# felipemcoelho/nf4-triton-dequantization

Hardware: AMD Instinct MI355X
Metric: dequantized elements/s (4096x4096 NF4->bf16, blocksize 64 / nested 256) (higher is better)
Workload: dtype f32

## Files before the change

nf4_triton_dequantization_amd/csrc/nf4_dequant.hip:

```cpp
#include <hip/hip_runtime.h>
#include <stdint.h>

#include "../../include/nf4_dequant.h"
#include "nf4_common.h"

namespace {

using namespace nf4dq;

enum Mode : int { kRef = 0, kSingle = 1, kBnb = 2, kBnbSingle = 3 };

struct Desc {
    const uint32_t* packed;
    const uint8_t* a1;
    const float* a2;
    const float* code2;
    u32x4* out;
    float offset;
    uint32_t nbytes;
    uint32_t tile_begin;
    uint32_t groups;
    FastDiv nb;
    FastDiv n2;
    FastDiv bpr;
    uint32_t blk_shift;
    uint32_t blk2_shift;
    uint32_t blk_base;
};

#ifndef NF4_FLAT_STAMPS
#define NF4_FLAT_STAMPS 0
#endif

template <int MAXB>
struct Batch {
    Desc d[MAXB];
    uint32_t count;
    uint32_t total_tiles;
#if NF4_FLAT_STAMPS
    unsigned long long* stamps;
#endif
};

#if NF4_FLAT_STAMPS
#define NF4_FSTAMP(slot_, val_)                                                                      \
    do {                                                                                             \
        __builtin_amdgcn_sched_barrier(0);                                                           \
        if (lane == 0) bt.stamps[(blockIdx.x * kFlatWaves + (threadIdx.x >> 6)) * 4u + (slot_)] = (val_); \
        __builtin_amdgcn_sched_barrier(0);                                                           \
    } while (0)
#define NF4_FNOW() __builtin_amdgcn_s_memrealtime()
#else
#define NF4_FSTAMP(slot_, val_) \
    do {                        \
    } while (0)
#define NF4_FNOW() 0ull
#endif

template <int DT>
__device__ __forceinline__ void store1(void* out, int64_t i, float x) {
    if constexpr (DT == NF4DQ_BF16) {
        reinterpret_cast<__bf16*>(out)[i] = (__bf16)x;
    } else if constexpr (DT == NF4DQ_F16) {
        reinterpret_cast<_Float16*>(out)[i] = (_Float16)opaque(x);
    } else {
        reinterpret_cast<float*>(out)[i] = x;
    }
}

#ifndef NF4_DQ_FLAT_WAVES
#define NF4_DQ_FLAT_WAVES 4
#endif
#ifndef NF4_DQ_U
#define NF4_DQ_U 4
#endif
#ifndef NF4_DQ_AUX_STORE
#define NF4_DQ_AUX_STORE 18
#endif
#ifndef NF4_DQ_AUX_LOAD
#define NF4_DQ_AUX_LOAD 2
#endif
#ifndef NF4_DQ_SCALE_FIRST
#define NF4_DQ_SCALE_FIRST 0
#endif
#ifndef NF4_DQ_SCALE_NT
#define NF4_DQ_SCALE_NT 0
#endif
#ifndef NF4_DQ_DECODE
#define NF4_DQ_DECODE 1
#endif
#ifndef NF4_DQ_SINGLE_FAST
#define NF4_DQ_SINGLE_FAST 1
#endif
#ifndef NF4_DQ_ABL_NOSCALE
#define NF4_DQ_ABL_NOSCALE 0
#endif



constexpr int kWg = 256;
constexpr int kFlatWaves = NF4_DQ_FLAT_WAVES;
constexpr int kFlatWg = 64 * kFlatWaves;
constexpr int kU = NF4_DQ_U;

constexpr int kAuxStore = NF4_DQ_AUX_STORE;
constexpr int kAuxLoad = NF4_DQ_AUX_LOAD;

template <int DT>
constexpr uint32_t out_bytes_per_packed_byte() { return DT == NF4DQ_F32 ? 8u : 4u; }
template <int DT>
constexpr uint32_t lane_bytes() { return DT == NF4DQ_F32 ? 2u : 4u; }
template <int DT>
constexpr uint32_t tile_bytes() { return 64u * lane_bytes<DT>() * kU; }

struct TileIn {
    uint32_t w[kU];
    uint32_t a1;
    float a2;
};

template <int DT>
__device__ __forceinline__ uint32_t tile_block(const Desc& D, uint32_t base, uint32_t lane) {
    constexpr uint32_t kTileBytes = tile_bytes<DT>();
    const uint32_t bsh = D.blk_shift;
    const uint32_t bpt = kTileBytes >> bsh;
    uint32_t g = (base >> bsh) + (bpt ? (lane & (bpt - 1u)) : 0u);
    const uint32_t nblk = (D.nbytes + (1u << bsh) - 1u) >> bsh;
    g = g < nblk ? g : nblk - 1u;
    return g + D.blk_base;
}

template <int DT, int MODE>
__device__ __forceinline__ TileIn tile_load(const Desc& D, __amdgpu_buffer_rsrc_t rp, uint32_t base, uint32_t lane) {
    constexpr uint32_t LB = lane_bytes<DT>();
    TileIn in;
    auto packed_loads = [&]() {
#pragma unroll
        for (int j = 0; j < kU; ++j) {
            const uint32_t off = base + 64u * LB * j + LB * lane;
            if constexpr (LB == 4) {
                in.w[j] = __builtin_amdgcn_raw_buffer_load_b32(rp, off, 0, kAuxLoad);
            } else {
                in.w[j] = __builtin_amdgcn_raw_buffer_load_b16(rp, off, 0, kAuxLoad);
            }
        }
    };
    if constexpr (!NF4_DQ_SCALE_FIRST) packed_loads();
    const uint32_t g = tile_block<DT>(D, base, lane);
    if constexpr (NF4_DQ_ABL_NOSCALE) {
        in.a1 = g & 255u;
        in.a2 = 0.01f;
    } else if constexpr (MODE == kRef) {
        const uint32_t r = fdiv(g, D.bpr);
        const uint32_t b = g - r * D.bpr.d;
        const uint8_t* pa1 = D.a1 + fmodu(g, D.nb);
        const float* pa2 = D.a2 + fmodu(r * D.groups + (b >> 2), D.n2);
        if constexpr (NF4_DQ_SCALE_NT) {
            in.a1 = __builtin_nontemporal_load(pa1);
            in.a2 = __builtin_nontemporal_load(pa2);
        } else {
            in.a1 = *pa1;
            in.a2 = *pa2;
        }
    } else if constexpr (MODE == kSingle) {
        const uint32_t r = fdiv(g, D.bpr);
        const uint32_t b = g - r * D.bpr.d;
        in.a2 = D.a2[r * D.n2.d + b];
    } else if constexpr (MODE == kBnb) {
        in.a1 = D.a1[g];
        in.a2 = D.a2[g >> D.blk2_shift];
    } else {
        in.a2 = D.a2[g];
    }
    if constexpr (NF4_DQ_SCALE_FIRST) packed_loads();
    return in;
}

template <int DT, int MODE>
__device__ __forceinline__ void tile_finish(const Desc& D, __amdgpu_buffer_rsrc_t ro, const float* lut,
                                            const TileIn& in, uint32_t base, uint32_t lane, const float* code2s) {
    float s;
    if constexpr (MODE == kRef) {
        s = ((float)in.a1 / 127.0f) * in.a2;
    } else if constexpr (MODE == kBnb) {
        s = code2s[in.a1] * in.a2 + D.offset;
    } else {
        s = in.a2;
    }
    const uint32_t bsh = D.blk_shift;
    constexpr uint32_t kOB = out_bytes_per_packed_byte<DT>();
    constexpr uint32_t LB = lane_bytes<DT>();
#pragma unroll
    for (int j = 0; j < kU; ++j) {
        const uint32_t rel = 64u * LB * j + LB * lane;
        const float sj = __shfl(s, (int)(rel >> bsh), 64);
        const uint32_t w = in.w[j];
        const uint32_t hi4 = (w >> 2) & 0x3C3C3C3Cu;
        const uint32_t lo4 = (w << 2) & 0x3C3C3C3Cu;
        const char* t = reinterpret_cast<const char*>(lut);
        float v[2 * LB];
#pragma unroll
        for (int k = 0; k < (int)LB; ++k) {
            v[2 * k] = *reinterpret_cast<const float*>(t + ((hi4 >> (8 * k)) & 0xFFu)) * sj;
            v[2 * k + 1] = *reinterpret_cast<const float*>(t + ((lo4 >> (8 * k)) & 0xFFu)) * sj;
        }
        const uint32_t ob = (base + rel) * kOB;
        if constexpr (DT == NF4DQ_F32) {
            u32x4 o = {__float_as_uint(v[0]), __float_as_uint(v[1]), __float_as_uint(v[2]), __float_as_uint(v[3])};
            __builtin_amdgcn_raw_buffer_store_b128(o, ro, ob, 0, kAuxStore);
        } else {
            u32x4 o = {pack2<DT>(v[0], v[1]), pack2<DT>(v[2], v[3]), pack2<DT>(v[4], v[5]), pack2<DT>(v[6], v[7])};
            __builtin_amdgcn_raw_buffer_store_b128(o, ro, ob, 0, kAuxStore);
        }
    }
}

typedef uint16_t __attribute__((may_alias)) u16_alias;
typedef uint32_t __attribute__((may_alias)) u32_alias;
typedef uint32_t u32x4_alias __attribute__((ext_vector_type(4), may_alias));

struct TblCtx {
    char* tbl;
    uint32_t tb;
    f32x2 c01;
};

template <int DT, int MODE>
__device__ __forceinline__ void tile_finish_tbl(const Desc& D, __amdgpu_buffer_rsrc_t ro, const TileIn& in,
                                                uint32_t base, uint32_t lane, const float* code2s,
                                                const TblCtx& c) {
    float s;
    if constexpr (MODE == kRef) {
        s = ((float)in.a1 / 127.0f) * in.a2;
    } else if constexpr (MODE == kBnb) {
        s = code2s[in.a1] * in.a2 + D.offset;
    } else {
        s = in.a2;
    }
    const uint32_t bsh = D.blk_shift;
    const uint32_t k = lane & 7u;
#pragma unroll
    for (int j = 0; j < kU; ++j) {
        const uint32_t rel = 256u * j + 4u * lane;
        const float sj = __shfl(s, (int)(rel >> bsh), 64);
        *reinterpret_cast<u32_alias*>(c.tbl + c.tb + 4u * k) = pack2<DT>(c.c01.x * sj, c.c01.y * sj);
        const uint32_t w = in.w[j];
        const uint32_t hb = (w >> 3) & 0x1E1E1E1Eu;
        const uint32_t lb = (w << 1) & 0x1E1E1E1Eu;
        uint32_t o[4];
#pragma unroll
        for (int b = 0; b < 4; ++b) {
            const uint32_t ah = __builtin_amdgcn_perm(hb, c.tb, 0x03020104u + b);
            const uint32_t al = __builtin_amdgcn_perm(lb, c.tb, 0x03020104u + b);
            const uint32_t vh = *reinterpret_cast<const u16_alias*>(c.tbl + ah);
            const uint32_t vl = *reinterpret_cast<const u16_alias*>(c.tbl + al);
            o[b] = vh | (vl << 16);
        }
        const u32x4 ov = {o[0], o[1], o[2], o[3]};
        __builtin_amdgcn_raw_buffer_store_b128(ov, ro, (base + rel) * 4u, 0, kAuxStore);
    }
}

template <int MAXB>
__device__ __forceinline__ uint32_t find_matrix(const Batch<MAXB>& bt, uint32_t t, uint32_t k) {
    if constexpr (MAXB > 1) {
        while (k + 1 < bt.count && t >= bt.d[k + 1].tile_begin) ++k;
    }
    return k;
}

struct Cursor {
    uint32_t t, k, base;
    bool valid;
};

template <int DT, int MAXB>
__device__ __forceinline__ Cursor cursor_at(const Batch<MAXB>& bt, uint32_t t, uint32_t k_hint) {
    constexpr uint32_t kTileBytes = tile_bytes<DT>();
    Cursor c;
    c.t = t;
    c.valid = t < bt.total_tiles;
    c.k = c.valid ? find_matrix(bt, t, k_hint) : k_hint;
    c.base = c.valid ? (t - bt.d[c.k].tile_begin) * kTileBytes : 0xFFFFF000u;
    return c;
}

template <int DT, int MAXB>
__device__ __forceinline__ void make_rsrcs(const Batch<MAXB>& bt, uint32_t k, __amdgpu_buffer_rsrc_t& rp,
                                           __amdgpu_buffer_rsrc_t& ro) {
    constexpr uint32_t kOB = out_bytes_per_packed_byte<DT>();
    rp = __builtin_amdgcn_make_buffer_rsrc((void*)bt.d[k].packed, 0, bt.d[k].nbytes, kRsrcFlags);
    ro = __builtin_amdgcn_make_buffer_rsrc((void*)bt.d[k].out, 0, bt.d[k].nbytes * kOB, kRsrcFlags);
}

template <int DT, int MODE, int MAXB>
__global__ __launch_bounds__(kFlatWg) void nf4_flat_kernel(const Batch<MAXB> bt) {
    __shared__ __attribute__((aligned(16))) float lut[16];
    __shared__ __attribute__((aligned(16))) float code2s[MODE == kBnb ? 256 : 1];
    constexpr bool kTbl = NF4_DQ_DECODE == 1 && DT != NF4DQ_F32;
    __shared__ __attribute__((aligned(256))) char tbl[kTbl ? kFlatWaves * 2048 : 4];
    const uint32_t lane = threadIdx.x & 63u;
#if NF4_FLAT_STAMPS
    const unsigned long long t_entry = NF4_FNOW();
    unsigned long long tiles_done = 0;
#endif
    const uint32_t t0 = __builtin_amdgcn_readfirstlane(blockIdx.x * kFlatWaves + (threadIdx.x >> 6));
    const uint32_t nwaves = gridDim.x * kFlatWaves;

    float c2w = 0.0f;
    if constexpr (MODE == kBnb) c2w = bt.d[0].code2[threadIdx.x & 255u];
    Cursor ca = cursor_at<DT>(bt, t0, 0u);
    __amdgpu_buffer_rsrc_t rpa, roa;
    make_rsrcs<DT>(bt, ca.k, rpa, roa);
    TileIn A = tile_load<DT, MODE>(bt.d[ca.k], rpa, ca.base, lane);
    const bool multi = !NF4_DQ_SINGLE_FAST || ca.t + nwaves < bt.total_tiles;
    if (multi) {
        const u32x4 z = {0u, 0u, 0u, 0u};
#pragma unroll
        for (int j = 0; j < kU; ++j) __builtin_amdgcn_raw_buffer_store_b128(z, roa, 0xFFFFF000u + 16u * j, 0, kAuxStore);
    }
    write_lut(lut);
    if constexpr (MODE == kBnb) {
        if constexpr (kFlatWg >= 256) {
            if (threadIdx.x < 256u) code2s[threadIdx.x] = c2w;
        } else {
            for (uint32_t i = threadIdx.x; i < 256u; i += kFlatWg) code2s[i] = bt.d[0].code2[i];
        }
    }
    __syncthreads();
    TblCtx tc{};
    if constexpr (kTbl) {
        tc.tbl = tbl;
        tc.tb = ((threadIdx.x >> 6) << 11) + ((lane >> 3) << 8);
        tc.c01 = *reinterpret_cast<const f32x2*>(lut + 2u * (lane & 7u));
    }
    if (!ca.valid) {
        NF4_FSTAMP(0, t_entry);
        NF4_FSTAMP(1, 0ull);
        NF4_FSTAMP(2, NF4_FNOW());
        NF4_FSTAMP(3, 0ull);
        return;
    }
    if (!multi) {
        if constexpr (kTbl) tile_finish_tbl<DT, MODE>(bt.d[ca.k], roa, A, ca.base, lane, code2s, tc);
        else tile_finish<DT, MODE>(bt.d[ca.k], roa, lut, A, ca.base, lane, code2s);
#if NF4_FLAT_STAMPS
        NF4_FSTAMP(1, NF4_FNOW());
        __builtin_amdgcn_s_waitcnt(0);
        NF4_FSTAMP(0, t_entry);
        NF4_FSTAMP(2, NF4_FNOW());
        NF4_FSTAMP(3, 1ull);
#endif
        return;
    }
    while (true) {
        const Cursor cb = cursor_at<DT>(bt, ca.t + nwaves, ca.k);
        __amdgpu_buffer_rsrc_t rpb = rpa, rob = roa;
        if (MAXB > 1 && cb.k != ca.k) make_rsrcs<DT>(bt, cb.k, rpb, rob);
        TileIn B = tile_load<DT, MODE>(bt.d[cb.k], rpb, cb.base, lane);
        if constexpr (kTbl) tile_finish_tbl<DT, MODE>(bt.d[ca.k], roa, A, ca.base, lane, code2s, tc);
        else tile_finish<DT, MODE>(bt.d[ca.k], roa, lut, A, ca.base, lane, code2s);
#if NF4_FLAT_STAMPS
        if (tiles_done == 0) NF4_FSTAMP(1, NF4_FNOW());
        ++tiles_done;
#endif
        if (!cb.valid) break;

        const Cursor cn = cursor_at<DT>(bt, cb.t + nwaves, cb.k);
        __amdgpu_buffer_rsrc_t rpn = rpb, ron = rob;
        if (MAXB > 1 && cn.k != cb.k) make_rsrcs<DT>(bt, cn.k, rpn, ron);
        A = tile_load<DT, MODE>(bt.d[cn.k], rpn, cn.base, lane);
        if constexpr (kTbl) tile_finish_tbl<DT, MODE>(bt.d[cb.k], rob, B, cb.base, lane, code2s, tc);
        else tile_finish<DT, MODE>(bt.d[cb.k], rob, lut, B, cb.base, lane, code2s);
#if NF4_FLAT_STAMPS
        ++tiles_done;
#endif
        if (!cn.valid) break;
        ca = cn;
        rpa = rpn;
        roa = ron;
    }
#if NF4_FLAT_STAMPS
    __builtin_amdgcn_s_waitcnt(0);
    NF4_FSTAMP(0, t_entry);
    NF4_FSTAMP(2, NF4_FNOW());
    NF4_FSTAMP(3, tiles_done);
#endif
}

struct RowsArgs {
    const uint8_t* packed;
    const uint8_t* a1;
    const float* a2;
    void* out;
    int64_t m, n, stride, cols_b;
    int64_t nb, n2, bpr, groups, rs;
};

template <int DT, int MODE>
__global__ __launch_bounds__(kWg) void nf4_rows_kernel(const RowsArgs A) {
    __shared__ __attribute__((aligned(16))) float lut[16];
    write_lut(lut);
    __syncthreads();
    const int64_t total = A.m * A.cols_b;
    for (int64_t i = (int64_t)blockIdx.x * kWg + threadIdx.x; i < total; i += (int64_t)gridDim.x * kWg) {
        const int64_t r = i / A.cols_b;
        const int64_t j = i - r * A.cols_b;
        const int64_t b = j >> 5;
        float s;
        if constexpr (MODE == kRef) {
            const float q = (float)A.a1[(r * A.bpr + b) % A.nb];
            s = (q / 127.0f) * A.a2[(r * A.groups + (b >> 2)) % A.n2];
        } else {
            s = A.a2[r * A.rs + b];
        }
        const uint32_t byte = A.packed[r * A.stride + j];
        const int64_t c = 2 * j;
        store1<DT>(A.out, r * A.n + c, lut[byte >> 4] * s);
        if (c + 1 < A.n) store1<DT>(A.out, r * A.n + c + 1, lut[byte & 15u] * s);
    }
}

struct ChunkArgs {
    const uint8_t* packed;
    const uint8_t* a1;
    const float* a2;
    void* out;
    uint64_t packed_len;
    uint64_t out_elems;
    uint32_t stride;
    uint32_t n;
    uint32_t chunks;
    FastDiv L;
    FastDiv bpr;
    uint32_t groups;
    FastDiv nb, n2;
    uint32_t rs;
};

constexpr uint32_t kDrop = 0xFFFFFFF0u;
constexpr int kAuxPiece = 0;
constexpr uint32_t kStageBytes = 4128;
constexpr uint32_t kStageDummy = 4112;

inline __device__ uint32_t range32(uint64_t v) { return v > 0x7FFFFFFFull ? 0x7FFFFFFFu : (uint32_t)v; }

inline __device__ uint32_t opaque_mul(uint32_t a, uint32_t b) {
    uint32_t r = a * b;
    asm("" : "+v"(r));
    return r;
}

template <int DT>
__device__ __forceinline__ void chunk_table_build(char* ctbl, uint32_t region, uint32_t lane, float sb) {
    uint32_t e[8];
#pragma unroll
    for (int k = 0; k < 8; ++k)
        e[k] = pack2<DT>(__uint_as_float(kNf4Bits[2 * k]) * sb, __uint_as_float(kNf4Bits[2 * k + 1]) * sb);
    u32x4_alias* dst = reinterpret_cast<u32x4_alias*>(ctbl + region + 32u * lane);
    dst[0] = u32x4{e[0], e[1], e[2], e[3]};
    dst[1] = u32x4{e[4], e[5], e[6], e[7]};
}

__device__ __forceinline__ void chunk_table_decode(const char* ctbl, uint32_t region, uint32_t w, uint32_t t,
                                                   uint32_t (&p)[4]) {
    t &= 63u;
    const uint32_t base = region + ((t >> 3) << 8);
    const uint32_t rep = __builtin_amdgcn_perm(0u, (t & 7u) << 5, 0x00000000u);
    const uint32_t hb = ((w >> 3) & 0x1E1E1E1Eu) | rep;
    const uint32_t lb = ((w << 1) & 0x1E1E1E1Eu) | rep;
#pragma unroll
    for (int b = 0; b < 4; ++b) {
        const uint32_t ah = __builtin_amdgcn_perm(hb, base, 0x03020104u + b);
        const uint32_t al = __builtin_amdgcn_perm(lb, base, 0x03020104u + b);
        const uint32_t vh = *reinterpret_cast<const u16_alias*>(ctbl + ah);
        const uint32_t vl = *reinterpret_cast<const u16_alias*>(ctbl + al);
        p[b] = vh | (vl << 16);
    }
}

template <int DT, int MODE>
__global__ __launch_bounds__(kWg) void nf4_chunk_dense_kernel(const ChunkArgs A) {
    __shared__ __attribute__((aligned(256))) char ctbl[4 * 2048];
    const uint32_t lane = threadIdx.x & 63u;
    const uint32_t cw = __builtin_amdgcn_readfirstlane((blockIdx.x * 4u + (threadIdx.x >> 6)) * 256u);
    const __amdgpu_buffer_rsrc_t rp =
        __builtin_amdgcn_make_buffer_rsrc((void*)A.packed, 0, (uint32_t)A.packed_len, kRsrcFlags);
    const __amdgpu_buffer_rsrc_t ro =
        __builtin_amdgcn_make_buffer_rsrc(A.out, 0, (uint32_t)(A.out_elems * 2u), kRsrcFlags);
    uint32_t w[4];
#pragma unroll
    for (int j = 0; j < 4; ++j)
        w[j] = __builtin_amdgcn_raw_buffer_load_b32(rp, 4u * (cw + 64u * j + lane), 0, kAuxLoad);
    __builtin_amdgcn_sched_barrier(0);
    const uint32_t cw0 = min(cw, A.chunks - 1u);
    const uint32_t r0 = fdiv(cw0, A.L);
    const uint32_t q0 = cw0 - r0 * A.L.d;
    const uint32_t cl = min(cw + 255u, A.chunks - 1u);
    const uint32_t rl = fdiv(cl, A.L);
    const uint32_t g0 = r0 * A.bpr.d + (q0 >> 3);
    const uint32_t gl = rl * A.bpr.d + ((cl - rl * A.L.d) >> 3);
    float sb;
    {
        const uint32_t g = min(g0 + lane, gl);
        const uint32_t r = fdiv(g, A.bpr);
        const uint32_t b = g - r * A.bpr.d;
        if constexpr (MODE == kRef) {
            const float q8 = (float)A.a1[fmodu(g, A.nb)];
            sb = (q8 / 127.0f) * A.a2[fmodu(opaque_mul(r, A.groups) + (b >> 2), A.n2)];
        } else {
            sb = A.a2[opaque_mul(r, A.rs) + b];
        }
    }
    uint32_t gsel[4];
    {
        uint32_t q = q0 + lane;
        const bool wrap = q >= A.L.d;
        q = wrap ? q - A.L.d : q;
        uint32_t gr = (wrap ? A.bpr.d : 0u) + r0 * A.bpr.d - g0;
#pragma unroll
        for (int j = 0; j < 4; ++j) {
            if (j) {
                q += 64u;
                const bool wj = q >= A.L.d;
                q = wj ? q - A.L.d : q;
                gr += wj ? A.bpr.d : 0u;
            }
            gsel[j] = gr + (q >> 3);
        }
    }
    const uint32_t region = (threadIdx.x >> 6) << 11;
    chunk_table_build<DT>(ctbl, region, lane, sb);
#pragma unroll
// ... 420 lines not shown
            d1[1] = u32x4{e[4], e[5], e[6], e[7]};
        }
    }
    const __amdgpu_buffer_rsrc_t ro =
        __builtin_amdgcn_make_buffer_rsrc(A.line, 0, 2u * (A.sa + A.elems), kRsrcFlags);
#pragma unroll
    for (int j = 0; j < 4; ++j) {
        const uint32_t cu = (uint32_t)max(W.c[j], 0);
        const uint32_t tA = min(W.gr[j] + (cu >> 6), 59u);
        const uint32_t to_blk = 64u - (cu & 63u), to_end = A.n - cu;
        const uint32_t ib_in = to_blk < to_end ? min(to_blk, 8u) : 8u, ib_end = min(to_end, 8u);
        uint32_t es, os;
        piece_codes<1, RE, TRI>(W.lo[j], W.hi[j], W.b[j], W.c[j], ib_in, ib_end, tA & 3u, W.lo2[j], W.hi2[j],
                                W.nb[j], es, os);
        const uint32_t base = region + ((tA >> 2) << 8);
        uint32_t p[4];
#pragma unroll
        for (int b = 0; b < 4; ++b) {
            const uint32_t ve = *reinterpret_cast<const u16_alias*>(ptbl + __builtin_amdgcn_perm(es, base, 0x03020104u + b));
            const uint32_t vo = *reinterpret_cast<const u16_alias*>(ptbl + __builtin_amdgcn_perm(os, base, 0x03020104u + b));
            p[b] = __builtin_amdgcn_perm(vo, ve, 0x05040100u);
        }
        const uint32_t k = kw + 64u * (uint32_t)j + lane;
        const int32_t f = W.fw + 8 * (64 * j + (int32_t)lane);
        const bool whole = f >= 0 && (uint32_t)f + 8u <= A.elems;
        const u32x4 o = {p[0], p[1], p[2], p[3]};
        __builtin_amdgcn_raw_buffer_store_b128(o, ro, whole ? 16u * k : kDrop, 0, kAuxStore);
        if (!whole && f < (int32_t)A.elems && f + 8 > 0) {
            const __amdgpu_buffer_rsrc_t rsp =
                __builtin_amdgcn_make_buffer_rsrc(A.out, 0, 2u * A.elems, kRsrcFlags);
#pragma unroll
            for (int i = 0; i < 8; ++i) {
                uint32_t oe = 2u * (uint32_t)(f + i);
                asm("" : "+v"(oe));
                __builtin_amdgcn_raw_buffer_store_b16((uint16_t)(p[i >> 1] >> (16 * (i & 1))), rsp, oe, 0,
                                                      kAuxPiece);
            }
        }
    }
}

constexpr uint32_t kPiece32Tbl = 12 * 256;

template <int MODE, int RE, bool TRI>
__global__ __launch_bounds__(kWg) void nf4_piece32_kernel(const PieceArgs A) {
    __shared__ __attribute__((aligned(256))) char ptbl[4 * kPiece32Tbl];
    const uint32_t lane = threadIdx.x & 63u;
    const uint32_t kw = __builtin_amdgcn_readfirstlane((blockIdx.x * 4u + (threadIdx.x >> 6)) * 256u);
    PieceWave<4, RE> W;
    if (!piece_wave<4, RE>(A, kw, lane, W)) return;
    const float sb = piece_scale<MODE>(A, W.g0, W.gl, lane);
    const uint32_t region = (threadIdx.x >> 6) * kPiece32Tbl;
    if (lane < 24u) {
        u32x4 e[4];
#pragma unroll
        for (int k = 0; k < 4; ++k)
            e[k] = u32x4{__float_as_uint(__uint_as_float(kNf4Bits[4 * k]) * sb),
                         __float_as_uint(__uint_as_float(kNf4Bits[4 * k + 1]) * sb),
                         __float_as_uint(__uint_as_float(kNf4Bits[4 * k + 2]) * sb),
                         __float_as_uint(__uint_as_float(kNf4Bits[4 * k + 3]) * sb)};
        u32x4_alias* d0 = reinterpret_cast<u32x4_alias*>(ptbl + region + ((lane >> 1) << 8) + ((lane & 1u) << 6));
#pragma unroll
        for (int k = 0; k < 4; ++k) d0[k] = e[k];
        if (lane >= 2u) {
            u32x4_alias* d1 = reinterpret_cast<u32x4_alias*>(ptbl + region + ((lane >> 1) << 8) - 256u + 128u +
                                                            ((lane & 1u) << 6));
#pragma unroll
            for (int k = 0; k < 4; ++k) d1[k] = e[k];
        }
    }
    const __amdgpu_buffer_rsrc_t ro =
        __builtin_amdgcn_make_buffer_rsrc(A.line, 0, 4u * (A.sa + A.elems), kRsrcFlags);
#pragma unroll
    for (int j = 0; j < 4; ++j) {
        const uint32_t cu = (uint32_t)max(W.c[j], 0);
        const uint32_t tA = min(W.gr[j] + (cu >> 6), 21u);
        const uint32_t to_blk = 64u - (cu & 63u), to_end = A.n - cu;
        const uint32_t ib_in = to_blk < to_end ? min(to_blk, 4u) : 4u, ib_end = min(to_end, 4u);
        uint32_t es, os;
        piece_codes<2, RE, TRI>(W.lo[j], W.hi[j], W.b[j], W.c[j], ib_in, ib_end, tA & 1u, W.lo2[j], W.hi2[j],
                                W.nb[j], es, os);
        const uint32_t base = region + ((tA >> 1) << 8);
        uint32_t p[4];
#pragma unroll
        for (int b = 0; b < 2; ++b) {
            p[2 * b] = *reinterpret_cast<const uint32_t*>(ptbl + __builtin_amdgcn_perm(es, base, 0x03020104u + b));
            p[2 * b + 1] = *reinterpret_cast<const uint32_t*>(ptbl + __builtin_amdgcn_perm(os, base, 0x03020104u + b));
        }
        const uint32_t k = kw + 64u * (uint32_t)j + lane;
        const int32_t f = W.fw + 4 * (64 * j + (int32_t)lane);
        const bool whole = f >= 0 && (uint32_t)f + 4u <= A.elems;
        const u32x4 o = {p[0], p[1], p[2], p[3]};
        __builtin_amdgcn_raw_buffer_store_b128(o, ro, whole ? 16u * k : kDrop, 0, kAuxStore);
        if (!whole && f < (int32_t)A.elems && f + 4 > 0) {
            const __amdgpu_buffer_rsrc_t rsp =
                __builtin_amdgcn_make_buffer_rsrc(A.out, 0, 4u * A.elems, kRsrcFlags);
#pragma unroll
            for (int i = 0; i < 4; ++i) {
                uint32_t oe = 4u * (uint32_t)(f + i);
                asm("" : "+v"(oe));
                __builtin_amdgcn_raw_buffer_store_b32(p[i], rsp, oe, 0, kAuxPiece);
            }
        }
    }
}

struct BnbBytesArgs {
    const uint8_t* packed;
    const uint8_t* a1;
    const float* code2;
    const float* a2;
    void* out;
    float offset;
    int64_t numel;
    int32_t blk_shift_elems, blk2_shift;
    int32_t single;
};

template <int DT>
__global__ __launch_bounds__(kWg) void nf4_bnb_bytes_kernel(const BnbBytesArgs A) {
    __shared__ __attribute__((aligned(16))) float lut[16];
    write_lut(lut);
    __syncthreads();
    const int64_t nbytes = (A.numel + 1) / 2;
    for (int64_t i = (int64_t)blockIdx.x * kWg + threadIdx.x; i < nbytes; i += (int64_t)gridDim.x * kWg) {
        const int64_t e = 2 * i;
        const int64_t blk = e >> A.blk_shift_elems;
        const float s = A.single ? A.a2[blk] : A.code2[A.a1[blk]] * A.a2[blk >> A.blk2_shift] + A.offset;
        const uint32_t byte = A.packed[i];
        store1<DT>(A.out, e, lut[byte >> 4] * s);
        if (e + 1 < A.numel) store1<DT>(A.out, e + 1, lut[byte & 15u] * s);
    }
}

inline int hip_rc(hipError_t e) { return e == hipSuccess ? NF4DQ_OK : NF4DQ_ERR_HIP_BASE + (int)e; }

inline bool valid_dtype(int32_t d) { return d == NF4DQ_F16 || d == NF4DQ_BF16 || d == NF4DQ_F32; }

inline bool aligned(const void* p, uintptr_t a) { return (reinterpret_cast<uintptr_t>(p) & (a - 1)) == 0; }

inline int ilog2(uint64_t v) {
    int s = 0;
    while ((uint64_t(1) << s) < v) ++s;
    return s;
}

constexpr nf4_launch_cfg kDefaultCfg = {4, 0, 1, 0};

#if NF4_FLAT_STAMPS
unsigned long long* g_stamps = nullptr;
#endif

int cu_count() {
    int dev = 0, cus = 0;
    if (hipGetDevice(&dev) != hipSuccess) return 256;
    if (hipDeviceGetAttribute(&cus, hipDeviceAttributeMultiprocessorCount, dev) != hipSuccess || cus <= 0) return 256;
    return cus;
}

template <int DT, int MODE, int MAXB>
void launch_one(const Batch<MAXB>& b, uint64_t blocks, hipStream_t st) {
    hipLaunchKernelGGL((nf4_flat_kernel<DT, MODE, MAXB>), dim3((unsigned)blocks), dim3(kFlatWg), 0, st, b);
}

template <int MAXB>
int launch_flat_batch(const Batch<MAXB>& bt, int dtype, int mode, const nf4_launch_cfg& cfg, hipStream_t st) {
    if (bt.count == 0) return NF4DQ_OK;
    const uint32_t tb = 64u * (dtype == NF4DQ_F32 ? 2u : 4u) * kU;
    Batch<MAXB> b = bt;
    uint32_t acc = 0;
    for (uint32_t i = 0; i < b.count; ++i) {
        b.d[i].tile_begin = acc;
        acc += (b.d[i].nbytes + tb - 1u) / tb;
    }
    b.total_tiles = acc;
    if (acc == 0) return NF4DQ_OK;
    uint64_t blocks = (acc + kFlatWaves - 1) / kFlatWaves;
    if (cfg.blocks_per_cu > 0) {
        const uint64_t cap = (uint64_t)cfg.blocks_per_cu * (uint64_t)cu_count();
        if (blocks > cap) blocks = cap;
    }
#if NF4_FLAT_STAMPS
    b.stamps = g_stamps;
#endif
#define NF4_D(DT_)                                                              \
    do {                                                                        \
        switch (mode) {                                                         \
            case kRef: launch_one<DT_, kRef, MAXB>(b, blocks, st); break;       \
            case kSingle: launch_one<DT_, kSingle, MAXB>(b, blocks, st); break; \
            case kBnb: launch_one<DT_, kBnb, MAXB>(b, blocks, st); break;       \
            default: launch_one<DT_, kBnbSingle, MAXB>(b, blocks, st); break;   \
        }                                                                       \
    } while (0)
    if (dtype == NF4DQ_BF16) NF4_D(NF4DQ_BF16);
    else if (dtype == NF4DQ_F16) NF4_D(NF4DQ_F16);
    else NF4_D(NF4DQ_F32);
#undef NF4_D
    return hip_rc(hipGetLastError());
}

inline unsigned rows_grid(int64_t work) {
    int64_t b = (work + kWg - 1) / kWg;
    if (b > 65536) b = 65536;
    if (b < 1) b = 1;
    return (unsigned)b;
}

int check_common(const uint8_t* packed, int64_t packed_len, const void* out, int32_t dtype, int64_t m, int64_t n) {
    if (!valid_dtype(dtype)) return NF4DQ_ERR_ARG;
    if (m < 0 || n < 0 || packed_len < 0) return NF4DQ_ERR_ARG;
    if (m == 0 || n == 0) return NF4DQ_OK;
    if (!packed || !out) return NF4DQ_ERR_ARG;
    if (packed_len % m) return NF4DQ_ERR_SHAPE;
    if (packed_len / m < (n + 1) / 2) return NF4DQ_ERR_SHAPE;
    return NF4DQ_OK;
}

constexpr int64_t kPieceBytes = int64_t(1) << 29;
constexpr int64_t kMaxFlatBlocks = int64_t(1) << 31;

bool flat_eligible(const uint8_t* packed, int64_t packed_len, const void* out, int64_t m, int64_t n) {
    return n % 64 == 0 && packed_len == m * (n / 2) && n / 2 < kPieceBytes && packed_len / 32 < kMaxFlatBlocks &&
           aligned(packed, 4) && aligned(out, 16);
}

inline int64_t piece_rows(int64_t n) { return (kPieceBytes - 1) / (n / 2); }

template <int MAXB>
int append_pieces(Batch<MAXB>& b, const Desc& proto, int64_t m, int64_t n, int32_t dtype, int mode,
                  hipStream_t st) {
    const int64_t rows = piece_rows(n);
    const int64_t ob = dtype == NF4DQ_F32 ? 4 * n : 2 * n;
    for (int64_t r0 = 0; r0 < m; r0 += rows) {
        const int64_t r1 = r0 + rows < m ? r0 + rows : m;
        Desc d = proto;
        d.packed = reinterpret_cast<const uint32_t*>(reinterpret_cast<const uint8_t*>(proto.packed) + r0 * (n / 2));
        d.out = reinterpret_cast<u32x4*>(reinterpret_cast<uint8_t*>(proto.out) + r0 * ob);
        d.nbytes = (uint32_t)((r1 - r0) * (n / 2));
        d.blk_base = (uint32_t)(r0 * (n / 64));
        d.tile_begin = b.total_tiles;
        b.d[b.count++] = d;
        b.total_tiles += (d.nbytes + 1023u) / 1024u;
        if (b.count == (uint32_t)MAXB || b.total_tiles > (1u << 30)) {
            const int rc = launch_flat_batch(b, dtype, mode, kDefaultCfg, st);
            if (rc) return rc;
            b.count = 0;
            b.total_tiles = 0;
        }
    }
    return NF4DQ_OK;
}

int launch_flat_matrix(const Desc& proto, int64_t m, int64_t n, int32_t dtype, int mode, const nf4_launch_cfg& cfg,
                       hipStream_t st) {
    const int64_t packed_len = m * (n / 2);
    if (packed_len < kPieceBytes) {
        Batch<1> b{};
        b.d[0] = proto;
        b.d[0].nbytes = (uint32_t)packed_len;
        b.count = 1;
        b.total_tiles = (uint32_t)((packed_len + 1023) / 1024);
        return launch_flat_batch(b, dtype, mode, cfg, st);
    }
    Batch<NF4DQ_BATCH_MAX> b{};
    const int rc = append_pieces(b, proto, m, n, dtype, mode, st);
    if (rc || b.count == 0) return rc;
    return launch_flat_batch(b, dtype, mode, kDefaultCfg, st);
}

Desc ref_desc(const uint8_t* packed, int64_t packed_len, const uint8_t* a1, int64_t nb, const float* a2,
              int64_t n2, void* out, int64_t n) {
    Desc d{};
    d.packed = reinterpret_cast<const uint32_t*>(packed);
    d.a1 = a1;
    d.a2 = a2;
    d.out = reinterpret_cast<u32x4*>(out);
    d.nbytes = packed_len < kPieceBytes ? (uint32_t)packed_len : 0u;
    const int64_t bpr = (n + 63) / 64;
    d.groups = (uint32_t)((bpr + 3) / 4);
    d.nb = make_fastdiv((uint32_t)(nb > (int64_t(1) << 31) ? (int64_t(1) << 31) : nb));
    d.n2 = make_fastdiv((uint32_t)(n2 > (int64_t(1) << 31) ? (int64_t(1) << 31) : n2));
    d.bpr = make_fastdiv((uint32_t)bpr);
    d.blk_shift = 5;
    return d;
}

bool chunk_args(ChunkArgs& A, const uint8_t* packed, int64_t packed_len, void* out, int32_t dtype, int64_t m,
                int64_t n) {
    const int64_t stride = packed_len / m;
    const int64_t L = ((n + 1) / 2 + 3) / 4;
    const int64_t bpr = (n + 63) / 64;
    const int64_t ob = dtype == NF4DQ_F32 ? 4 : 2;
    const int64_t span = 256 / L + 2;
    const int64_t lim = int64_t(1) << 31;
    if (m * L >= lim - 1024 || m * bpr >= lim || n >= (int64_t(1) << 28) || span * stride >= lim ||
        span * n * ob >= lim || !aligned(out, (uintptr_t)ob))
        return false;
    A.packed = packed;
    A.out = out;
    A.packed_len = (uint64_t)packed_len;
    A.out_elems = (uint64_t)(m * n);
    A.stride = (uint32_t)stride;
    A.n = (uint32_t)n;
    A.chunks = (uint32_t)(m * L);
    A.L = make_fastdiv((uint32_t)L);
    A.bpr = make_fastdiv((uint32_t)bpr);
    A.groups = (uint32_t)((bpr + 3) / 4);
    return true;
}

template <int DT, int MODE, int LW>
void launch_chunks_lw(const ChunkArgs& A, int sw, unsigned g, hipStream_t st) {
    if (sw == 16) hipLaunchKernelGGL((nf4_chunk_kernel<DT, MODE, LW, 16>), dim3(g), dim3(kWg), 0, st, A);
    else hipLaunchKernelGGL((nf4_chunk_kernel<DT, MODE, LW, 4>), dim3(g), dim3(kWg), 0, st, A);
}

bool dense_eligible(const ChunkArgs& A, int32_t dtype) {
    return dtype != NF4DQ_F32 && A.L.d >= 64u && A.stride == 4u * A.L.d && A.n % 8u == 0 && aligned(A.packed, 4) &&
           aligned(A.out, 16) && A.chunks < (1u << 27);
}

bool piece_eligible(const ChunkArgs& A, int32_t dtype) {
    const uint64_t half = (A.n + 1u) / 2u;
    const uint64_t rows = A.out_elems / A.n;
    const uint64_t ob = dtype == NF4DQ_F32 ? 4u : 2u;
    if (A.stride != half && dtype != NF4DQ_F32 && A.n % 8u == 0 && aligned(A.out, 16)) return false;
    return A.stride >= half && A.packed_len == rows * A.stride && A.n >= 512u &&
           ob * (A.out_elems + 64u) < (uint64_t(1) << 31) && A.packed_len + 8u < (uint64_t(1) << 31);
}

template <int MODE, int DT, int RE, bool TRI>
void launch_pieces_k(const PieceArgs& P, unsigned g, hipStream_t st) {
    if constexpr (DT == NF4DQ_F32) hipLaunchKernelGGL((nf4_piece32_kernel<MODE, RE, TRI>), dim3(g), dim3(kWg), 0, st, P);
// ... 158 lines not shown
    A.out = out;
    A.m = m;
    A.n = n;
    A.stride = packed_len / m;
    A.cols_b = (n + 1) / 2;
    A.bpr = bpr;
    A.rs = rs;
    const unsigned g = rows_grid(m * A.cols_b);
    if (out_dtype == NF4DQ_BF16) hipLaunchKernelGGL((nf4_rows_kernel<NF4DQ_BF16, kSingle>), dim3(g), dim3(kWg), 0, st, A);
    else if (out_dtype == NF4DQ_F16) hipLaunchKernelGGL((nf4_rows_kernel<NF4DQ_F16, kSingle>), dim3(g), dim3(kWg), 0, st, A);
    else hipLaunchKernelGGL((nf4_rows_kernel<NF4DQ_F32, kSingle>), dim3(g), dim3(kWg), 0, st, A);
    return hip_rc(hipGetLastError());
}

int nf4_dequant_ref_batched(const nf4_matrix_desc* descs, int32_t count, int32_t out_dtype, void* hip_stream) {
    hipStream_t st = reinterpret_cast<hipStream_t>(hip_stream);
    if (count < 0 || (count > 0 && !descs)) return NF4DQ_ERR_ARG;
    if (!valid_dtype(out_dtype)) return NF4DQ_ERR_ARG;
    for (int32_t i = 0; i < count; ++i) {
        const nf4_matrix_desc& d = descs[i];
        int rc = check_common(d.packed, d.packed_len, d.out, out_dtype, d.m, d.n);
        if (rc) return rc;
        if (d.m == 0 || d.n == 0) continue;
        if (!d.absmax_q || !d.absmax2 || d.nb <= 0 || d.n2 <= 0) return NF4DQ_ERR_ARG;
    }
    Batch<NF4DQ_BATCH_MAX> b{};
    b.count = 0;
    b.total_tiles = 0;
    for (int32_t i = 0; i < count; ++i) {
        const nf4_matrix_desc& d = descs[i];
        if (d.m == 0 || d.n == 0) continue;
        if (!flat_eligible(d.packed, d.packed_len, d.out, d.m, d.n)) {
            int rc = ref_impl(d.packed, d.packed_len, d.absmax_q, d.nb, d.absmax2, d.n2, d.out, out_dtype, d.m, d.n,
                              kDefaultCfg, st);
            if (rc) return rc;
            continue;
        }
        const int rc = append_pieces(b, ref_desc(d.packed, d.packed_len, d.absmax_q, d.nb, d.absmax2, d.n2, d.out,
                                                 d.n), d.m, d.n, out_dtype, kRef, st);
        if (rc) return rc;
    }
    if (b.count) return launch_flat_batch(b, out_dtype, kRef, kDefaultCfg, st);
    return NF4DQ_OK;
}

static int bnb_common(const uint8_t* packed, const uint8_t* a1, int64_t nb, const float* code2, const float* a2,
                      int64_t n2, float offset, void* out, int32_t dtype, int64_t numel, int32_t blocksize,
                      int32_t blocksize2, bool single, hipStream_t st) {
    if (!valid_dtype(dtype)) return NF4DQ_ERR_ARG;
    if (numel < 0) return NF4DQ_ERR_ARG;
    if (numel == 0) return NF4DQ_OK;
    if (!packed || !out || !a2) return NF4DQ_ERR_ARG;
    if (blocksize < 64 || (blocksize & (blocksize - 1))) return NF4DQ_ERR_ARG;
    const int64_t nblk = (numel + blocksize - 1) / blocksize;
    if (nb < nblk) return NF4DQ_ERR_SHAPE;
    if (!single) {
        if (!a1 || !code2) return NF4DQ_ERR_ARG;
        if (blocksize2 <= 0 || (blocksize2 & (blocksize2 - 1))) return NF4DQ_ERR_ARG;
        if (n2 < (nblk + blocksize2 - 1) / blocksize2) return NF4DQ_ERR_SHAPE;
    }
    const int mode = single ? kBnbSingle : kBnb;
    if (numel % 8 == 0 && nblk < kMaxFlatBlocks && blocksize <= (1 << 28) && aligned(packed, 4) && aligned(out, 16)) {
        const int64_t nbytes = numel / 2;
        const int64_t row = nbytes < kPieceBytes ? nbytes : kPieceBytes / 2;
        Desc d{};
        d.packed = reinterpret_cast<const uint32_t*>(packed);
        d.a1 = a1;
        d.a2 = a2;
        d.code2 = code2;
        d.out = reinterpret_cast<u32x4*>(out);
        d.offset = offset;
        d.blk_shift = (uint32_t)ilog2((uint64_t)blocksize / 2);
        d.blk2_shift = single ? 0u : (uint32_t)ilog2((uint64_t)blocksize2);
        if (nbytes < kPieceBytes) {
            Batch<1> b{};
            b.d[0] = d;
            b.d[0].nbytes = (uint32_t)nbytes;
            b.count = 1;
            b.total_tiles = (uint32_t)((nbytes + 1023) / 1024);
            return launch_flat_batch(b, dtype, mode, kDefaultCfg, st);
        }
        Batch<NF4DQ_BATCH_MAX> b{};
        const int64_t ob = dtype == NF4DQ_F32 ? 8 : 4;
        for (int64_t p0 = 0; p0 < nbytes; p0 += row) {
            Desc x = d;
            const int64_t len = nbytes - p0 < row ? nbytes - p0 : row;
            x.packed = reinterpret_cast<const uint32_t*>(packed + p0);
            x.out = reinterpret_cast<u32x4*>(reinterpret_cast<uint8_t*>(out) + p0 * ob);
            x.nbytes = (uint32_t)len;
            x.blk_base = (uint32_t)(p0 >> d.blk_shift);
            x.tile_begin = b.total_tiles;
            b.d[b.count++] = x;
            b.total_tiles += (uint32_t)((len + 1023) / 1024);
            if (b.count == NF4DQ_BATCH_MAX) {
                const int rc = launch_flat_batch(b, dtype, mode, kDefaultCfg, st);
                if (rc) return rc;
                b.count = 0;
                b.total_tiles = 0;
            }
        }
        return b.count ? launch_flat_batch(b, dtype, mode, kDefaultCfg, st) : NF4DQ_OK;
    }
    BnbBytesArgs A{};
    A.packed = packed;
    A.a1 = a1;
    A.code2 = code2;
    A.a2 = a2;
    A.out = out;
    A.offset = offset;
    A.numel = numel;
    A.blk_shift_elems = ilog2((uint64_t)blocksize);
    A.blk2_shift = single ? 0 : ilog2((uint64_t)blocksize2);
    A.single = single ? 1 : 0;
    const unsigned g = rows_grid((numel + 1) / 2);
    if (dtype == NF4DQ_BF16) hipLaunchKernelGGL((nf4_bnb_bytes_kernel<NF4DQ_BF16>), dim3(g), dim3(kWg), 0, st, A);
    else if (dtype == NF4DQ_F16) hipLaunchKernelGGL((nf4_bnb_bytes_kernel<NF4DQ_F16>), dim3(g), dim3(kWg), 0, st, A);
    else hipLaunchKernelGGL((nf4_bnb_bytes_kernel<NF4DQ_F32>), dim3(g), dim3(kWg), 0, st, A);
    return hip_rc(hipGetLastError());
}

int nf4_dequant_bnb(const uint8_t* packed, const uint8_t* absmax_q, int64_t nb, const float* code2,
                    const float* absmax2, int64_t n2, float offset, void* out, int32_t out_dtype, int64_t numel,
                    int32_t blocksize, int32_t blocksize2, void* hip_stream) {
    return bnb_common(packed, absmax_q, nb, code2, absmax2, n2, offset, out, out_dtype, numel, blocksize, blocksize2,
                      false, reinterpret_cast<hipStream_t>(hip_stream));
}

int nf4_dequant_bnb_single(const uint8_t* packed, const float* absmax, int64_t nabs, void* out, int32_t out_dtype,
                           int64_t numel, int32_t blocksize, void* hip_stream) {
    return bnb_common(packed, nullptr, nabs, nullptr, absmax, 0, 0.0f, out, out_dtype, numel, blocksize, 1, true,
                      reinterpret_cast<hipStream_t>(hip_stream));
}

const char* nf4_strerror(int code) {
    switch (code) {
        case NF4DQ_OK: return "ok";
        case NF4DQ_ERR_ARG: return "invalid argument (null pointer, dtype or negative size)";
        case NF4DQ_ERR_SHAPE: return "shape mismatch (packed weight / absmax cannot be viewed as the reference does)";
        case NF4DQ_ERR_TOO_LARGE: return "matrix too large for one launch";
        case NF4DQ_ERR_SPLITK_TIMEOUT:
            return "fused GEMM split-K hand-off timed out (some outputs are NaN; workspace re-zeroed)";
        default: break;
    }
    if (code >= NF4DQ_ERR_HIP_BASE) return hipGetErrorString((hipError_t)(code - NF4DQ_ERR_HIP_BASE));
    return "unknown error";
}

const char* nf4_version(void) { return "nf4dq 0.2.0 gfx950"; }

#if NF4_FLAT_STAMPS
void nf4_dbg_set_stamps(void* buf) { g_stamps = reinterpret_cast<unsigned long long*>(buf); }
#endif

}
```

Measured before the change: 2285 billion.

## Replace two-stage tile ping-pong with configurable ring of in-flight tile loads

The flat kernel's A/B double-buffer loop becomes a ring of kRing (default 4) outstanding tile loads per wave, so more global loads are in flight while earlier tiles are decoded and stored. Cursor values are forced uniform with readfirstlane, the single-tile fast path and dummy stores are reworked, and table setup is deferred until after the ring's loads are issued. It also caches the CU count on the host and adds an optional hook for the grid-size rule. The deeper ring raises VGPR pressure, which may lower occupancy, and with default settings most waves in this workload own only one or a few tiles.

```diff
diff --git a/nf4_triton_dequantization_amd/csrc/nf4_dequant.hip b/nf4_triton_dequantization_amd/csrc/nf4_dequant.hip
--- a/nf4_triton_dequantization_amd/csrc/nf4_dequant.hip
+++ b/nf4_triton_dequantization_amd/csrc/nf4_dequant.hip
@@ -1,5 +1,7 @@
 #include <hip/hip_runtime.h>
 #include <stdint.h>
+
+#include <atomic>
 
 #include "../../include/nf4_dequant.h"
 #include "nf4_common.h"
@@ -89,11 +91,17 @@
 #ifndef NF4_DQ_DECODE
 #define NF4_DQ_DECODE 1
 #endif
-#ifndef NF4_DQ_SINGLE_FAST
-#define NF4_DQ_SINGLE_FAST 1
-#endif
 #ifndef NF4_DQ_ABL_NOSCALE
 #define NF4_DQ_ABL_NOSCALE 0
+#endif
+#ifndef NF4_DQ_RING
+#define NF4_DQ_RING 4
+#endif
+#ifndef NF4_DQ_RING_DUMMY
+#define NF4_DQ_RING_DUMMY 0
+#endif
+#ifndef NF4_DQ_RULE_HOOK
+#define NF4_DQ_RULE_HOOK 0
 #endif
 
 
@@ -102,6 +110,8 @@
 constexpr int kFlatWaves = NF4_DQ_FLAT_WAVES;
 constexpr int kFlatWg = 64 * kFlatWaves;
 constexpr int kU = NF4_DQ_U;
+constexpr int kRing = NF4_DQ_RING;
+static_assert(kRing >= 2 && kRing <= 4, "ring depth: (kRing - 1) * (kU + 2 + kU) must fit the 6-bit vmcnt");
 
 constexpr int kAuxStore = NF4_DQ_AUX_STORE;
 constexpr int kAuxLoad = NF4_DQ_AUX_LOAD;
@@ -115,7 +125,7 @@
 
 struct TileIn {
     uint32_t w[kU];
-    uint32_t a1;
+    uint8_t a1;
     float a2;
 };
 
@@ -148,7 +158,7 @@
     if constexpr (!NF4_DQ_SCALE_FIRST) packed_loads();
     const uint32_t g = tile_block<DT>(D, base, lane);
     if constexpr (NF4_DQ_ABL_NOSCALE) {
-        in.a1 = g & 255u;
+        in.a1 = (uint8_t)(g & 255u);
         in.a2 = 0.01f;
     } else if constexpr (MODE == kRef) {
         const uint32_t r = fdiv(g, D.bpr);
@@ -225,7 +235,7 @@
     f32x2 c01;
 };
 
-template <int DT, int MODE>
+template <int DT, int MODE, bool RING = false>
 __device__ __forceinline__ void tile_finish_tbl(const Desc& D, __amdgpu_buffer_rsrc_t ro, const TileIn& in,
                                                 uint32_t base, uint32_t lane, const float* code2s,
                                                 const TblCtx& c) {
@@ -243,7 +253,9 @@
     for (int j = 0; j < kU; ++j) {
         const uint32_t rel = 256u * j + 4u * lane;
         const float sj = __shfl(s, (int)(rel >> bsh), 64);
-        *reinterpret_cast<u32_alias*>(c.tbl + c.tb + 4u * k) = pack2<DT>(c.c01.x * sj, c.c01.y * sj);
+        float e0 = c.c01.x * sj, e1 = c.c01.y * sj;
+        if constexpr (RING) asm("" : "+v"(e0));
+        *reinterpret_cast<u32_alias*>(c.tbl + c.tb + 4u * k) = pack2<DT>(e0, e1);
         const uint32_t w = in.w[j];
         const uint32_t hb = (w >> 3) & 0x1E1E1E1Eu;
         const uint32_t lb = (w << 1) & 0x1E1E1E1Eu;
@@ -271,17 +283,20 @@
 
 struct Cursor {
     uint32_t t, k, base;
-    bool valid;
 };
 
+__device__ __forceinline__ uint32_t tile_after(uint32_t t, uint32_t stride, uint32_t tend) {
+    return t < tend ? t + stride : t;
+}
+
 template <int DT, int MAXB>
-__device__ __forceinline__ Cursor cursor_at(const Batch<MAXB>& bt, uint32_t t, uint32_t k_hint) {
+__device__ __forceinline__ Cursor cursor_at(const Batch<MAXB>& bt, uint32_t t, uint32_t tend, uint32_t k_hint) {
     constexpr uint32_t kTileBytes = tile_bytes<DT>();
     Cursor c;
-    c.t = t;
-    c.valid = t < bt.total_tiles;
-    c.k = c.valid ? find_matrix(bt, t, k_hint) : k_hint;
-    c.base = c.valid ? (t - bt.d[c.k].tile_begin) * kTileBytes : 0xFFFFF000u;
+    c.t = __builtin_amdgcn_readfirstlane(t);
+    const bool valid = c.t < tend;
+    c.k = valid ? find_matrix(bt, c.t, k_hint) : k_hint;
+    c.base = __builtin_amdgcn_readfirstlane(valid ? (c.t - bt.d[c.k].tile_begin) * kTileBytes : 0xFFFFF000u);
     return c;
 }
 
@@ -305,45 +320,52 @@
     unsigned long long tiles_done = 0;
 #endif
     const uint32_t t0 = __builtin_amdgcn_readfirstlane(blockIdx.x * kFlatWaves + (threadIdx.x >> 6));
-    const uint32_t nwaves = gridDim.x * kFlatWaves;
+    const uint32_t stride = gridDim.x * kFlatWaves;
+    const uint32_t tend = bt.total_tiles;
 
     float c2w = 0.0f;
     if constexpr (MODE == kBnb) c2w = bt.d[0].code2[threadIdx.x & 255u];
-    Cursor ca = cursor_at<DT>(bt, t0, 0u);
-    __amdgpu_buffer_rsrc_t rpa, roa;
-    make_rsrcs<DT>(bt, ca.k, rpa, roa);
-    TileIn A = tile_load<DT, MODE>(bt.d[ca.k], rpa, ca.base, lane);
-    const bool multi = !NF4_DQ_SINGLE_FAST || ca.t + nwaves < bt.total_tiles;
-    if (multi) {
-        const u32x4 z = {0u, 0u, 0u, 0u};
-#pragma unroll
-        for (int j = 0; j < kU; ++j) __builtin_amdgcn_raw_buffer_store_b128(z, roa, 0xFFFFF000u + 16u * j, 0, kAuxStore);
-    }
-    write_lut(lut);
-    if constexpr (MODE == kBnb) {
-        if constexpr (kFlatWg >= 256) {
-            if (threadIdx.x < 256u) code2s[threadIdx.x] = c2w;
-        } else {
-            for (uint32_t i = threadIdx.x; i < 256u; i += kFlatWg) code2s[i] = bt.d[0].code2[i];
-        }
-    }
-    __syncthreads();
+    Cursor c[kRing];
+    __amdgpu_buffer_rsrc_t rp[kRing], ro[kRing];
+    TileIn in[kRing];
+    c[0] = cursor_at<DT>(bt, t0, tend, 0u);
+    make_rsrcs<DT>(bt, c[0].k, rp[0], ro[0]);
+    in[0] = tile_load<DT, MODE>(bt.d[c[0].k], rp[0], c[0].base, lane);
     TblCtx tc{};
-    if constexpr (kTbl) {
-        tc.tbl = tbl;
-        tc.tb = ((threadIdx.x >> 6) << 11) + ((lane >> 3) << 8);
-        tc.c01 = *reinterpret_cast<const f32x2*>(lut + 2u * (lane & 7u));
-    }
-    if (!ca.valid) {
-        NF4_FSTAMP(0, t_entry);
-        NF4_FSTAMP(1, 0ull);
-        NF4_FSTAMP(2, NF4_FNOW());
-        NF4_FSTAMP(3, 0ull);
-        return;
-    }
-    if (!multi) {
-        if constexpr (kTbl) tile_finish_tbl<DT, MODE>(bt.d[ca.k], roa, A, ca.base, lane, code2s, tc);
-        else tile_finish<DT, MODE>(bt.d[ca.k], roa, lut, A, ca.base, lane, code2s);
+    auto tables = [&]() {
+        write_lut(lut);
+        if constexpr (MODE == kBnb) {
+            if constexpr (kFlatWg >= 256) {
+                if (threadIdx.x < 256u) code2s[threadIdx.x] = c2w;
+            } else {
+                for (uint32_t i = threadIdx.x; i < 256u; i += kFlatWg) code2s[i] = bt.d[0].code2[i];
+            }
+        }
+        __syncthreads();
+        if constexpr (kTbl) {
+            tc.tbl = tbl;
+            tc.tb = ((threadIdx.x >> 6) << 11) + ((lane >> 3) << 8);
+            tc.c01 = *reinterpret_cast<const f32x2*>(lut + 2u * (lane & 7u));
+        }
+    };
+    auto finish = [&](int s) {
+        if constexpr (kTbl) tile_finish_tbl<DT, MODE>(bt.d[c[s].k], ro[s], in[s], c[s].base, lane, code2s, tc);
+        else tile_finish<DT, MODE>(bt.d[c[s].k], ro[s], lut, in[s], c[s].base, lane, code2s);
+    };
+    auto ring_finish = [&](int s) {
+        if constexpr (kTbl) tile_finish_tbl<DT, MODE, true>(bt.d[c[s].k], ro[s], in[s], c[s].base, lane, code2s, tc);
+        else tile_finish<DT, MODE>(bt.d[c[s].k], ro[s], lut, in[s], c[s].base, lane, code2s);
+    };
+    if (!(tile_after(t0, stride, tend) < tend)) {
+        tables();
+        if (!(c[0].t < tend)) {
+            NF4_FSTAMP(0, t_entry);
+            NF4_FSTAMP(1, 0ull);
+            NF4_FSTAMP(2, NF4_FNOW());
+            NF4_FSTAMP(3, 0ull);
+            return;
+        }
+        finish(0);
 #if NF4_FLAT_STAMPS
         NF4_FSTAMP(1, NF4_FNOW());
         __builtin_amdgcn_s_waitcnt(0);
@@ -353,32 +375,48 @@
 #endif
         return;
     }
-    while (true) {
-        const Cursor cb = cursor_at<DT>(bt, ca.t + nwaves, ca.k);
-        __amdgpu_buffer_rsrc_t rpb = rpa, rob = roa;
-        if (MAXB > 1 && cb.k != ca.k) make_rsrcs<DT>(bt, cb.k, rpb, rob);
-        TileIn B = tile_load<DT, MODE>(bt.d[cb.k], rpb, cb.base, lane);
-        if constexpr (kTbl) tile_finish_tbl<DT, MODE>(bt.d[ca.k], roa, A, ca.base, lane, code2s, tc);
-        else tile_finish<DT, MODE>(bt.d[ca.k], roa, lut, A, ca.base, lane, code2s);
+    asm volatile("" : "+s"(c[0].k));
+#pragma unroll
+    for (int s = 1; s < kRing; ++s) {
+#if NF4_DQ_RING_DUMMY
+        const u32x4 z = {0u, 0u, 0u, 0u};
+#pragma unroll
+        for (int j = 0; j < kU; ++j)
+            __builtin_amdgcn_raw_buffer_store_b128(z, ro[0], 0xFFFFF000u + 16u * j, 0, kAuxStore);
+#endif
+        c[s] = cursor_at<DT>(bt, tile_after(c[s - 1].t, stride, tend), tend, c[s - 1].k);
+        rp[s] = rp[s - 1];
+        ro[s] = ro[s - 1];
+        if (MAXB > 1 && c[s].k != c[s - 1].k) make_rsrcs<DT>(bt, c[s].k, rp[s], ro[s]);
+        in[s] = tile_load<DT, MODE>(bt.d[c[s].k], rp[s], c[s].base, lane);
+    }
+    tables();
+    while ((uint64_t)c[0].t + (uint64_t)kRing * stride < tend) {
+#pragma unroll
+        for (int s = 0; s < kRing; ++s) {
+            const int sp = (s + kRing - 1) % kRing;
+            ring_finish(s);
+#if NF4_FLAT_STAMPS
+            if (tiles_done == 0) NF4_FSTAMP(1, NF4_FNOW());
+            ++tiles_done;
+#endif
+            const Cursor cn = cursor_at<DT>(bt, tile_after(c[sp].t, stride, tend), tend, c[sp].k);
+            __amdgpu_buffer_rsrc_t rpn = rp[sp], ron = ro[sp];
+            if (MAXB > 1 && cn.k != c[sp].k) make_rsrcs<DT>(bt, cn.k, rpn, ron);
+            c[s] = cn;
+            rp[s] = rpn;
+            ro[s] = ron;
+            in[s] = tile_load<DT, MODE>(bt.d[cn.k], rpn, cn.base, lane);
+        }
+    }
+#pragma unroll
+    for (int s = 0; s < kRing; ++s) {
+        if (s && !(c[s].t < tend)) break;
+        ring_finish(s);
 #if NF4_FLAT_STAMPS
         if (tiles_done == 0) NF4_FSTAMP(1, NF4_FNOW());
         ++tiles_done;
 #endif
-        if (!cb.valid) break;
-
-        const Cursor cn = cursor_at<DT>(bt, cb.t + nwaves, cb.k);
-        __amdgpu_buffer_rsrc_t rpn = rpb, ron = rob;
-        if (MAXB > 1 && cn.k != cb.k) make_rsrcs<DT>(bt, cn.k, rpn, ron);
-        A = tile_load<DT, MODE>(bt.d[cn.k], rpn, cn.base, lane);
-        if constexpr (kTbl) tile_finish_tbl<DT, MODE>(bt.d[cb.k], rob, B, cb.base, lane, code2s, tc);
-        else tile_finish<DT, MODE>(bt.d[cb.k], rob, lut, B, cb.base, lane, code2s);
-#if NF4_FLAT_STAMPS
-        ++tiles_done;
-#endif
-        if (!cn.valid) break;
-        ca = cn;
-        rpa = rpn;
-        roa = ron;
     }
 #if NF4_FLAT_STAMPS
     __builtin_amdgcn_s_waitcnt(0);
@@ -1105,10 +1143,29 @@
 #endif
 
 int cu_count() {
+    static std::atomic<int> cached[64];
     int dev = 0, cus = 0;
     if (hipGetDevice(&dev) != hipSuccess) return 256;
+    const bool slot = dev >= 0 && dev < 64;
+    if (slot && (cus = cached[dev].load(std::memory_order_relaxed)) > 0) return cus;
     if (hipDeviceGetAttribute(&cus, hipDeviceAttributeMultiprocessorCount, dev) != hipSuccess || cus <= 0) return 256;
+    if (slot) cached[dev].store(cus, std::memory_order_relaxed);
     return cus;
+}
+
+#if NF4_DQ_RULE_HOOK
+int g_hook_tpw = 1, g_hook_wpc = 0;
+#endif
+
+uint32_t flat_tiles_per_wave(uint32_t tiles) {
+#if NF4_DQ_RULE_HOOK
+    if (g_hook_tpw > 0) return (uint32_t)g_hook_tpw;
+    const uint64_t cap = (uint64_t)(g_hook_wpc > 0 ? g_hook_wpc : 1) * (uint64_t)cu_count();
+    return tiles > cap ? (uint32_t)((tiles + cap - 1) / cap) : 1u;
+#else
+    (void)tiles;
+    return 1u;
+#endif
 }
 
 template <int DT, int MODE, int MAXB>
@@ -1132,6 +1189,10 @@
     if (cfg.blocks_per_cu > 0) {
         const uint64_t cap = (uint64_t)cfg.blocks_per_cu * (uint64_t)cu_count();
         if (blocks > cap) blocks = cap;
+    } else {
+        const uint32_t tpw = flat_tiles_per_wave(acc);
+        const uint64_t waves = (acc + tpw - 1) / tpw;
+        blocks = (waves + kFlatWaves - 1) / kFlatWaves;
     }
 #if NF4_FLAT_STAMPS
     b.stamps = g_stamps;
@@ -1596,4 +1657,11 @@
 void nf4_dbg_set_stamps(void* buf) { g_stamps = reinterpret_cast<unsigned long long*>(buf); }
 #endif
 
-}
+#if NF4_DQ_RULE_HOOK
+void nf4_dbg_set_flat_rule(int tiles_per_wave, int waves_per_cu) {
+    g_hook_tpw = tiles_per_wave;
+    g_hook_wpc = waves_per_cu;
+}
+#endif
+
+}
```

Result: no change. 2270 billion (-0.7%).
